# C-X-Lu/Replication-of-Minute-Frequency-Factor

Measured on AMD Instinct MI355X. Metric: factor stock-days/sec (whole node) + % of HBM roofline, 5000×240min×2500d, higher is better.
Workload: dtype f64

## Files before the change

### replication-of-minute-frequency-factor_amd/csrc/mff_group.h

```cpp
#pragma once
#include <hip/hip_runtime.h>
#include <stdint.h>

#include "mff_wave.h"

namespace mff {
namespace g16 {

__device__ __forceinline__ int gi() { return (int)(threadIdx.x & 15u); }
__device__ __forceinline__ int gbase() { return (int)(threadIdx.x & 48u); }

constexpr int QP_XOR1 = 0xB1;
constexpr int QP_XOR2 = 0x4E;
constexpr int ROW_SHR = 0x110;
constexpr int ROW_SHL = 0x100;
constexpr int ROW_MIRROR = 0x140;
constexpr int ROW_HALF_MIRROR = 0x141;
constexpr int K = 16;

template <int CTRL>
__device__ __forceinline__ int dpp_i(int x) {
  return __builtin_amdgcn_mov_dpp(x, CTRL, 0xF, 0xF, true);
}
template <int CTRL>
__device__ __forceinline__ uint32_t dpp_u(uint32_t x) { return (uint32_t)dpp_i<CTRL>((int)x); }
template <int CTRL>
__device__ __forceinline__ float dpp_f(float x) { return __int_as_float(dpp_i<CTRL>(__float_as_int(x))); }
template <int CTRL>
__device__ __forceinline__ double dpp_d(double x) {
  const uint64_t b = dbits(x);
  const uint32_t lo = (uint32_t)dpp_i<CTRL>((int)(uint32_t)b);
  const uint32_t hi = (uint32_t)dpp_i<CTRL>((int)(uint32_t)(b >> 32));
  return bitsd(((uint64_t)hi << 32) | lo);
}
template <int CTRL>
__device__ __forceinline__ uint64_t dpp_u64(uint64_t b) {
  const uint32_t lo = (uint32_t)dpp_i<CTRL>((int)(uint32_t)b);
  const uint32_t hi = (uint32_t)dpp_i<CTRL>((int)(uint32_t)(b >> 32));
  return ((uint64_t)hi << 32) | lo;
}

template <int CTRL>
__device__ __forceinline__ float dppT(float x) { return dpp_f<CTRL>(x); }
template <int CTRL>
__device__ __forceinline__ double dppT(double x) { return dpp_d<CTRL>(x); }
template <int CTRL>
__device__ __forceinline__ uint32_t dppT(uint32_t x) { return dpp_u<CTRL>(x); }

__device__ __forceinline__ double gsum(double x) {
  x += dpp_d<QP_XOR1>(x);
  x += dpp_d<QP_XOR2>(x);
  x += dpp_d<ROW_HALF_MIRROR>(x);
  x += dpp_d<ROW_MIRROR>(x);
  return x;
}
__device__ __forceinline__ double gprod(double x) {
  x *= dpp_d<QP_XOR1>(x);
  x *= dpp_d<QP_XOR2>(x);
  x *= dpp_d<ROW_HALF_MIRROR>(x);
  x *= dpp_d<ROW_MIRROR>(x);
  return x;
}
__device__ __forceinline__ int gsum_i(int x) {
  x += dpp_i<QP_XOR1>(x);
  x += dpp_i<QP_XOR2>(x);
  x += dpp_i<ROW_HALF_MIRROR>(x);
  x += dpp_i<ROW_MIRROR>(x);
  return x;
}
__device__ __forceinline__ uint32_t gsum_u(uint32_t x) { return (uint32_t)gsum_i((int)x); }
__device__ __forceinline__ int gmin_i(int x) {
  x = min(x, dpp_i<QP_XOR1>(x));
  x = min(x, dpp_i<QP_XOR2>(x));
  x = min(x, dpp_i<ROW_HALF_MIRROR>(x));
  x = min(x, dpp_i<ROW_MIRROR>(x));
  return x;
}
__device__ __forceinline__ int gmax_i(int x) {
  x = max(x, dpp_i<QP_XOR1>(x));
  x = max(x, dpp_i<QP_XOR2>(x));
  x = max(x, dpp_i<ROW_HALF_MIRROR>(x));
  x = max(x, dpp_i<ROW_MIRROR>(x));
  return x;
}
__device__ __forceinline__ bool gany(bool b) { return gmax_i(b ? 1 : 0) != 0; }

__device__ __forceinline__ double gscan_incl(double x) {
  x += dpp_d<ROW_SHR + 1>(x);
  x += dpp_d<ROW_SHR + 2>(x);
  x += dpp_d<ROW_SHR + 4>(x);
  x += dpp_d<ROW_SHR + 8>(x);
  return x;
}
__device__ __forceinline__ uint32_t gscan_incl_u(uint32_t x) {
  x += dpp_u<ROW_SHR + 1>(x);
  x += dpp_u<ROW_SHR + 2>(x);
  x += dpp_u<ROW_SHR + 4>(x);
  x += dpp_u<ROW_SHR + 8>(x);
  return x;
}
__device__ __forceinline__ double gscan_excl(double x) { return dpp_d<ROW_SHR + 1>(gscan_incl(x)); }
__device__ __forceinline__ uint32_t gscan_excl_u(uint32_t x) { return dpp_u<ROW_SHR + 1>(gscan_incl_u(x)); }

template <typename T>
__device__ __forceinline__ void carry_left(T v, bool h, T& cv, bool& ch) {
  uint32_t hh = h ? 1u : 0u;
#pragma unroll
  for (int step = 0; step < 4; ++step) {
    T ov;
    uint32_t oh;
    if (step == 0) { ov = dppT<ROW_SHR + 1>(v); oh = dpp_u<ROW_SHR + 1>(hh); }
    if (step == 1) { ov = dppT<ROW_SHR + 2>(v); oh = dpp_u<ROW_SHR + 2>(hh); }
    if (step == 2) { ov = dppT<ROW_SHR + 4>(v); oh = dpp_u<ROW_SHR + 4>(hh); }
    if (step == 3) { ov = dppT<ROW_SHR + 8>(v); oh = dpp_u<ROW_SHR + 8>(hh); }
    if (!hh && oh) { v = ov; hh = 1u; }
  }
  cv = dppT<ROW_SHR + 1>(v);
  ch = dpp_u<ROW_SHR + 1>(hh) != 0u;
}
template <typename T>
__device__ __forceinline__ void carry_right(T v, bool h, T& cv, bool& ch) {
  uint32_t hh = h ? 1u : 0u;
#pragma unroll
  for (int step = 0; step < 4; ++step) {
    T ov;
    uint32_t oh;
    if (step == 0) { ov = dppT<ROW_SHL + 1>(v); oh = dpp_u<ROW_SHL + 1>(hh); }
    if (step == 1) { ov = dppT<ROW_SHL + 2>(v); oh = dpp_u<ROW_SHL + 2>(hh); }
    if (step == 2) { ov = dppT<ROW_SHL + 4>(v); oh = dpp_u<ROW_SHL + 4>(hh); }
    if (step == 3) { ov = dppT<ROW_SHL + 8>(v); oh = dpp_u<ROW_SHL + 8>(hh); }
    if (!hh && oh) { v = ov; hh = 1u; }
  }
  cv = dppT<ROW_SHL + 1>(v);
  ch = dpp_u<ROW_SHL + 1>(hh) != 0u;
}

__device__ __forceinline__ int bpermi(int src_lane, int v) { return __builtin_amdgcn_ds_bpermute(src_lane << 2, v); }
__device__ __forceinline__ float bpermf(int src_lane, float v) { return __int_as_float(bpermi(src_lane, __float_as_int(v))); }
__device__ __forceinline__ uint32_t bpermu(int src_lane, uint32_t v) { return (uint32_t)bpermi(src_lane, (int)v); }
__device__ __forceinline__ double bpermd(int src_lane, double v) {
  const uint64_t b = dbits(v);
  const uint32_t lo = (uint32_t)bpermi(src_lane, (int)(uint32_t)b);
  const uint32_t hi = (uint32_t)bpermi(src_lane, (int)(uint32_t)(b >> 32));
  return bitsd(((uint64_t)hi << 32) | lo);
}

__device__ __forceinline__ uint32_t blend_u(bool c, uint32_t a, uint32_t b) {
  const uint32_t m = 0u - (uint32_t)c;
  return (a & m) | (b & ~m);
}
__device__ __forceinline__ uint32_t pick(const uint32_t (&x)[K], int k) {
  uint32_t t = x[0];
#pragma unroll
  for (int j = 1; j < K; ++j) t = blend_u(k == j, x[j], t);
  return t;
}
__device__ __forceinline__ float pick(const float (&x)[K], int k) {
  uint32_t t = __float_as_uint(x[0]);
#pragma unroll
  for (int j = 1; j < K; ++j) t = blend_u(k == j, __float_as_uint(x[j]), t);
  return __uint_as_float(t);
}
__device__ __forceinline__ uint64_t pick(const uint64_t (&x)[K], int k) {
  uint32_t lo = (uint32_t)x[0], hi = (uint32_t)(x[0] >> 32);
#pragma unroll
  for (int j = 1; j < K; ++j) {
    lo = blend_u(k == j, (uint32_t)x[j], lo);
    hi = blend_u(k == j, (uint32_t)(x[j] >> 32), hi);
  }
  return ((uint64_t)hi << 32) | lo;
}
__device__ __forceinline__ float gval(const float (&x)[K], int m) {
  return bpermf(gbase() + (m >> 4), pick(x, m & 15));
}
__device__ __forceinline__ uint32_t gvalu(const uint32_t (&x)[K], int m) {
  return bpermu(gbase() + (m >> 4), pick(x, m & 15));
}
template <int M>
__device__ __forceinline__ float gvalc(const float (&x)[K]) {
  return bpermf(gbase() + (M >> 4), x[M & 15]);
}
__device__ __forceinline__ bool gpres(uint32_t pb, int m) {
  return (bpermu(gbase() + (m >> 4), pb) >> (m & 15)) & 1u;
}

__device__ __forceinline__ uint32_t present_bits(uint32_t pb, int k) { return (uint32_t)((int32_t)(pb << (31 - k)) >> 31); }
__device__ __forceinline__ uint32_t absent_bits(uint32_t pb, int k) { return ~present_bits(pb, k); }

__device__ __forceinline__ uint32_t rmask(int lo, int hi) {
  const int b0 = 16 * gi();
  int a = lo - b0, b = hi - b0;
  if (a < 0) a = 0;
  if (b > 15) b = 15;
  if (b < a) return 0u;
  return ((0xFFFFu >> (15 - b)) >> a) << a;
}
__device__ __forceinline__ int gfirst(uint32_t m) {
  const int v = m ? 16 * gi() + (int)__builtin_ctz(m) : (1 << 20);
  const int r = gmin_i(v);
  return r == (1 << 20) ? -1 : r;
}
__device__ __forceinline__ int glast(uint32_t m) {
  return gmax_i(m ? 16 * gi() + 31 - (int)__builtin_clz(m) : -1);
}
__device__ __forceinline__ int gcount(uint32_t m) { return gsum_i(__builtin_popcount(m)); }
__device__ __forceinline__ uint32_t gmax_u(uint32_t x) {
  x = max(x, dpp_u<QP_XOR1>(x));
  x = max(x, dpp_u<QP_XOR2>(x));
  x = max(x, dpp_u<ROW_HALF_MIRROR>(x));
  x = max(x, dpp_u<ROW_MIRROR>(x));
  return x;
}
__device__ __forceinline__ uint32_t gmin_u(uint32_t x) {
  x = min(x, dpp_u<QP_XOR1>(x));
  x = min(x, dpp_u<QP_XOR2>(x));
  x = min(x, dpp_u<ROW_HALF_MIRROR>(x));
  x = min(x, dpp_u<ROW_MIRROR>(x));
  return x;
}

constexpr int QP_XOR3 = 0x1B;
constexpr int ROW_ROR8 = 0x128;

template <int CTRL>
__device__ __forceinline__ uint32_t dpp_full(uint32_t x) {
  return (uint32_t)__builtin_amdgcn_mov_dpp((int)x, CTRL, 0xF, 0xF, false);
}
__device__ __forceinline__ uint32_t swz_xor4(uint32_t x) {
  return (uint32_t)__builtin_amdgcn_ds_swizzle((int)x, 0x1F | (4 << 10));
}
template <int M>
__device__ __forceinline__ uint32_t gpartner(uint32_t x) {
  return (uint32_t)__builtin_amdgcn_ds_swizzle((int)x, 0x1F | (M << 10));
}
template <int M, int LB, bool FLIP>
__device__ __forceinline__ void gcross(uint32_t (&a)[K]) {
  const uint32_t bound = (gi() & LB) == 0 ? 0u : 0xFFFFFFFFu;
  uint32_t p[K];
#pragma unroll
  for (int k = 0; k < K; ++k) p[k] = gpartner<M>(a[FLIP ? K - 1 - k : k]);
#pragma unroll
  for (int k = 0; k < K; ++k) asm("v_med3_u32 %0, %1, %2, %3" : "=v"(a[k]) : "v"(a[k]), "v"(p[k]), "v"(bound));
}
template <int J, bool FLIP>
__device__ __forceinline__ void glocal(uint32_t (&a)[K]) {
#pragma unroll
  for (int k = 0; k < K; ++k) {
    const int o = FLIP ? (k ^ (2 * J - 1)) : (k ^ J);
    if (o > k) {
      const uint32_t x = a[k], y = a[o];
      a[k] = min(x, y);
      a[o] = max(x, y);
    }
  }
}
__device__ __forceinline__ void glocal_tail(uint32_t (&a)[K]) {
  glocal<8, false>(a);
  glocal<4, false>(a);
  glocal<2, false>(a);
  glocal<1, false>(a);
}
__device__ __forceinline__ void gsort16_lane(uint32_t (&a)[K]) {
  constexpr int8_t net[60][2] = {
      {0, 13}, {1, 12}, {2, 15}, {3, 14}, {4, 8}, {5, 6}, {7, 11}, {9, 10},
      {0, 5}, {1, 7}, {2, 9}, {3, 4}, {6, 13}, {8, 14}, {10, 15}, {11, 12},
      {0, 1}, {2, 3}, {4, 5}, {6, 8}, {7, 9}, {10, 11}, {12, 13}, {14, 15},
      {0, 2}, {1, 3}, {4, 10}, {5, 11}, {6, 7}, {8, 9}, {12, 14}, {13, 15},
      {1, 2}, {3, 12}, {4, 6}, {5, 7}, {8, 10}, {9, 11}, {13, 14},
      {1, 4}, {2, 6}, {5, 8}, {7, 10}, {9, 13}, {11, 14},
      {2, 4}, {3, 6}, {9, 12}, {11, 13},
// ... 22 lines not shown
```

### replication-of-minute-frequency-factor_amd/csrc/mff_stage1g.hip

```cpp
#include <stdlib.h>
#include <string.h>

#include <type_traits>

#include "../../include/mff.h"
#include "mff_group.h"
#include "mff_fmath.h"
#include "mff_stats.h"
#include "mff_internal.h"

namespace mff {

int launch_w64(const float* const fld[5], const uint32_t* valid, int S, int D, const int32_t* ids, int nf,
               double* val, uint8_t* state, double* pdfq, const int* list, const int* list_count,
               uint32_t fam_mask, int list_grid, hipStream_t st, uint32_t* lvl_count = nullptr,
               uint64_t* lvl_key = nullptr, uint8_t* lvl_w = nullptr);
int launch_serial(const float* const fld[5], const uint32_t* valid, int S, int D, const int8_t* row,
                  uint32_t fam, double* val, uint8_t* state, const uint32_t* ord_th, hipStream_t st);

constexpr int kGIter = 1;
constexpr int kGWaves = 5;
constexpr int kExactGrid = 1024;

namespace g16 {

constexpr int NB = 256;

struct GArgs {
  const float* fld[5];
  const uint32_t* mask;
  double* val;
  uint8_t* state;
  double* pdfq;
  uint32_t* lvl_count;
  uint64_t* lvl_key;
  uint8_t* lvl_w;
  int* fb_list;
  int* fb_count;
  uint32_t fam_exact;
  uint32_t* ord_th;
  int S, D;
  uint32_t fam;
  int8_t row[NF];
};

struct Res {
  double r[4];
  uint32_t st;
  __device__ __forceinline__ void put(int f, double x, uint32_t s) {
    if (gi() == (f & 15)) {
      const int q = f >> 4;
      r[q] = x;
      st = (st & ~(0xFFu << (8 * q))) | (s << (8 * q));
    }
  }
  __device__ __forceinline__ void val(int f, double x) { put(f, x, MFF_STATE_VALUE); }
  __device__ __forceinline__ void null(int f) { put(f, 0.0, MFF_STATE_NULL); }
};

__device__ __forceinline__ double gmin_d(double x) {
  x = fmin(x, dpp_d<QP_XOR1>(x));
  x = fmin(x, dpp_d<QP_XOR2>(x));
  x = fmin(x, dpp_d<ROW_HALF_MIRROR>(x));
  x = fmin(x, dpp_d<ROW_MIRROR>(x));
  return x;
}
__device__ __forceinline__ double gmax_d(double x) {
  x = fmax(x, dpp_d<QP_XOR1>(x));
  x = fmax(x, dpp_d<QP_XOR2>(x));
  x = fmax(x, dpp_d<ROW_HALF_MIRROR>(x));
  x = fmax(x, dpp_d<ROW_MIRROR>(x));
  return x;
}

__device__ __forceinline__ void opaque(float& x) { asm("" : "+v"(x)); }
__device__ __forceinline__ void opaque(double& x) { asm("" : "+v"(x)); }
__device__ __forceinline__ void opaque(uint32_t& x) { asm("" : "+v"(x)); }
template <typename T>
__device__ __forceinline__ void fresh(T (&x)[K]) {
#pragma unroll
  for (int k = 0; k < K; ++k) opaque(x[k]);
}

__device__ __forceinline__ void lds_fence() {
  __builtin_amdgcn_fence(__ATOMIC_RELEASE, "wavefront");
  __builtin_amdgcn_wave_barrier();
  __builtin_amdgcn_fence(__ATOMIC_ACQUIRE, "wavefront");
}

__device__ __forceinline__ uint32_t xor_lane(uint32_t x, int lj) { return (uint32_t)__shfl_xor((int)x, lj, 16); }
__device__ __forceinline__ uint64_t xor_lane(uint64_t x, int lj) {
  const uint32_t lo = xor_lane((uint32_t)x, lj), hi = xor_lane((uint32_t)(x >> 32), lj);
  return ((uint64_t)hi << 32) | lo;
}

template <typename T>
__device__ __forceinline__ void gsort256(T (&a)[K]) {
  const int g = gi();
#pragma unroll
  for (int size = 2; size <= 256; size <<= 1) {
#pragma unroll
    for (int j = size >> 1; j > 0; j >>= 1) {
      if (j >= 16) {
        const int lj = j >> 4;
        const bool lower = (g & lj) == 0;
        const bool up = ((16 * g) & size) == 0;
#pragma unroll
        for (int k = 0; k < K; ++k) {
          const T p = xor_lane(a[k], lj);
          const T mn = a[k] < p ? a[k] : p, mx = a[k] < p ? p : a[k];
          a[k] = (lower == up) ? mn : mx;
        }
      } else {
#pragma unroll
        for (int k = 0; k < K; ++k) {
          if ((k & j) == 0) {
            const bool up = ((16 * g + k) & size) == 0;
            const T x = a[k], y = a[k | j];
            const T mn = x < y ? x : y, mx = x < y ? y : x;
            a[k] = up ? mn : mx;
            a[k | j] = up ? mx : mn;
          }
        }
      }
    }
  }
}

[[maybe_unused]] constexpr uint32_t G_HL = F_OLS | F_MOMH;
constexpr uint32_t G_ORD = F_ORD | F_ORDV;
constexpr uint32_t G_LVL = F_LVL | F_PDF;
constexpr uint32_t kGroups[2] = {G_ORD, G_LVL};
constexpr uint32_t G_OL = G_ORD | G_LVL;

template <uint32_t SET>
__global__ __launch_bounds__(256, kGWaves) void k_stage1g(GArgs a) {
  constexpr int SW = (SET & F_OLS) ? 2 * NB : 2 * NBAR;
  __shared__ __attribute__((aligned(16))) uint64_t scratch[16][SW / 2 + 8];
  const int lane = lane_id();
  const int wave = threadIdx.x >> 6;
  const int grp = lane >> 4;
  const int g = gi();
  const int gb = gbase();
  uint64_t* scr = scratch[wave * 4 + grp];
  double* scr_d = reinterpret_cast<double*>(scr);
  const uint32_t fam = a.fam & SET;
  const int ntile = (a.S + 16 * kGIter - 1) / (16 * kGIter);
  const int d = blockIdx.x / ntile;
  const int s0 = (blockIdx.x % ntile) * (16 * kGIter);
  const size_t plane = (size_t)a.D * a.S;

  for (int it = 0; it < kGIter; ++it) {
    const int s = s0 + it * 16 + wave * 4 + grp;
    const bool act = s < a.S;
    const size_t sd = (size_t)d * a.S + (act ? s : 0);
    const bool ln = act && g < 15;

    uint32_t pb = 0;
    if (ln) {
      const uint32_t w = a.mask[sd * 8 + (g >> 1)];
      pb = (w >> (16 * (g & 1))) & 0xFFFFu;
    }
    const int n = gcount(pb);
    Res R;
    R.r[0] = R.r[1] = R.r[2] = R.r[3] = 0.0;
    R.st = 0u;
    double qv = qnan();
    uint32_t emitL = 0u, emitB = 0u;
    float emitC = 1.0f;

    if (n > 0) {
      float o[K], h[K], lo[K], c[K];
      uint32_t v[K];
      auto load = [&](int f, float (&x)[K], float dflt) {
        if (ln) {
          const float4* p4 = reinterpret_cast<const float4*>(a.fld[f] + sd * NBAR + 16 * g);
#pragma unroll
          for (int q = 0; q < 4; ++q) {
            const float4 t = p4[q];
            x[4 * q + 0] = t.x; x[4 * q + 1] = t.y; x[4 * q + 2] = t.z; x[4 * q + 3] = t.w;
          }
        } else {
#pragma unroll
          for (int k = 0; k < K; ++k) x[k] = dflt;
        }
      };
      constexpr uint32_t needO = F_SEG | F_MOMR | F_TRD;
      constexpr uint32_t needHL = F_OLS | F_MOMH;
      constexpr uint32_t needC = F_SEG | F_MOMR | F_SUMC | F_CORR | F_LVL | F_PDF | F_TRD;
      constexpr uint32_t needV = F_ORD | F_MOMV | F_SUMC | F_SUMV | F_CORR | F_LVL | F_PDF | F_ORDV | F_TRD;
      static_assert(!(needO & ~kFieldFams[0]) && !(needHL & ~(kFieldFams[1] & kFieldFams[2])) &&
                        !(needC & ~kFieldFams[3]) && !(needV & ~kFieldFams[4]),
                    "k_stage1g loads a field for a family kFieldFams does not list");
      auto loadv = [&](uint32_t (&x)[K]) {
        if (ln) {
          const uint4* p4 = reinterpret_cast<const uint4*>(a.fld[4] + sd * NBAR + 16 * g);
#pragma unroll
          for (int q = 0; q < 4; ++q) {
            const uint4 t = p4[q];
            x[4 * q + 0] = t.x; x[4 * q + 1] = t.y; x[4 * q + 2] = t.z; x[4 * q + 3] = t.w;
          }
#pragma unroll
          for (int k = 0; k < K; ++k) x[k] &= present_bits(pb, k);
        } else {
#pragma unroll
          for (int k = 0; k < K; ++k) x[k] = 0u;
        }
      };
      auto sanitize = [&](float (&x)[K], float dflt) {
#pragma unroll
        for (int k = 0; k < K; ++k) {
          if (dflt == 0.0f)
            x[k] = bitsf(fbits(x[k] + 0.0f) & present_bits(pb, k));
          else
            x[k] = ((pb >> k) & 1u) ? x[k] + 0.0f : dflt;
        }
      };
      if (fam & needHL) {
        load(1, h, 1.0f);
        load(2, lo, 1.0f);
        sanitize(h, 1.0f);
        sanitize(lo, 1.0f);
      }
      const int fb = gfirst(pb), lb = glast(pb);

      if (fam & F_OLS) {
        const double x0a = (double)gval(lo, fb), y0a = (double)gval(h, fb);
        const float ln0 = dpp_f<ROW_SHL + 1>(lo[0]), hn0 = dpp_f<ROW_SHL + 1>(h[0]);
        const uint32_t pn0 = dpp_u<ROW_SHL + 1>(pb) & 1u;
        double tx = 0, ty = 0, txx = 0, tyy = 0, txy = 0, q15x = 0, q15y = 0, q15xx = 0, q15yy = 0, q15xy = 0;
        uint32_t tpk = 0, q15pk = 0;
#pragma unroll
        for (int k = 0; k < K; ++k) {
          const bool pk = (pb >> k) & 1u;
          const bool pnx = (k < 15) ? ((pb >> (k + 1)) & 1u) : (pn0 != 0u);
          const float lnx = (k < 15) ? lo[k + 1] : ln0, hnx = (k < 15) ? h[k + 1] : hn0;
          const double dx = pk ? (double)lo[k] - x0a : 0.0, dy = pk ? (double)h[k] - y0a : 0.0;
          const uint32_t pkv = (pk ? 1u : 0u) | ((pk && pnx && lo[k] != lnx) ? 0x100u : 0u) |
                               ((pk && pnx && h[k] != hnx) ? 0x10000u : 0u);
          tx += dx; ty += dy; txx += dx * dx; tyy += dy * dy; txy += dx * dy; tpk += pkv;
          if (k == 15) { q15x = dx; q15y = dy; q15xx = dx * dx; q15yy = dy * dy; q15xy = dx * dy; q15pk = pkv; }
        }
        double Rx = gscan_excl(tx), Ry = gscan_excl(ty), Rxx = gscan_excl(txx), Ryy = gscan_excl(tyy),
               Rxy = gscan_excl(txy);
        uint32_t Rpk = gscan_excl_u(tpk);
        const double E15x = Rx + tx, E15y = Ry + ty, E15xx = Rxx + txx, E15yy = Ryy + tyy, E15xy = Rxy + txy;
        const uint32_t E15pk = Rpk + tpk;
        double x0 = x0a, y0 = y0a;
        opaque(x0);
        opaque(y0);
#pragma unroll
        for (int k = 0; k < K; ++k) { opaque(lo[k]); opaque(h[k]); }
        double H1x = 0, H1y = 0, H1xx = 0, H1yy = 0, H1xy = 0, H2x = 0, H2y = 0, H2xx = 0, H2yy = 0, H2xy = 0;
        uint32_t H1pk = 0, H2pk = 0;
        double sq = 0, scs = 0, scr = 0, bsum = 0, blast = 0;
        int lastT = -1, wq = 0;
        uint32_t wmask = 0;
#pragma unroll
        for (int k = 0; k < K; ++k) {
          const bool pk = (pb >> k) & 1u;
          const bool pnx = (k < 15) ? ((pb >> (k + 1)) & 1u) : (pn0 != 0u);
          const float lnx = (k < 15) ? lo[k + 1] : ln0, hnx = (k < 15) ? h[k + 1] : hn0;
          const double dx = pk ? (double)lo[k] - x0 : 0.0, dy = pk ? (double)h[k] - y0 : 0.0;
          const uint32_t chx = (pk && pnx && lo[k] != lnx) ? 1u : 0u;
          const uint32_t chy = (pk && pnx && h[k] != hnx) ? 1u : 0u;
          Rx += dx; Ry += dy; Rxx += dx * dx; Ryy += dy * dy; Rxy += dx * dy;
          Rpk += (pk ? 1u : 0u) | (chx << 8) | (chy << 16);
          double bx, by, bxx, byy, bxy;
          uint32_t bpk;
          if (k >= 2) {
            const int src = gb + (g >= 3 ? g - 3 : 0);
            bx = bpermd(src, H2x); by = bpermd(src, H2y); bxx = bpermd(src, H2xx);
            byy = bpermd(src, H2yy); bxy = bpermd(src, H2xy); bpk = bpermu(src, H2pk);
            if (g < 3) { bx = by = bxx = byy = bxy = 0.0; bpk = 0u; }
          } else {
            const int src = gb + (g >= 4 ? g - 4 : 0);
            const double ex = (k == 0) ? E15x - q15x : E15x, ey = (k == 0) ? E15y - q15y : E15y;
            const double exx = (k == 0) ? E15xx - q15xx : E15xx, eyy = (k == 0) ? E15yy - q15yy : E15yy;
            const double exy = (k == 0) ? E15xy - q15xy : E15xy;
            const uint32_t epk = (k == 0) ? E15pk - q15pk : E15pk;
            bx = bpermd(src, ex); by = bpermd(src, ey); bxx = bpermd(src, exx);
            byy = bpermd(src, eyy); bxy = bpermd(src, exy); bpk = bpermu(src, epk);
            if (g < 4) { bx = by = bxx = byy = bxy = 0.0; bpk = 0u; }
          }
          H2x = H1x; H2y = H1y; H2xx = H1xx; H2yy = H1yy; H2xy = H1xy; H2pk = H1pk;
          H1x = Rx; H1y = Ry; H1xx = Rxx; H1yy = Ryy; H1xy = Rxy; H1pk = Rpk;
          const int t = 16 * g + k;
          const uint32_t cnt = (Rpk & 0xffu) - (bpk & 0xffu);
          const uint32_t cxw = ((Rpk >> 8) & 0xffu) - ((bpk >> 8) & 0xffu) - chx;
          const uint32_t cyw = ((Rpk >> 16) & 0xffu) - ((bpk >> 16) & 0xffu) - chy;
          const bool okw = ln && t >= 49 && cnt == 50u;
          if (okw) {
            const double Sx = Rx - bx, Sy = Ry - by, Sxx = Rxx - bxx, Syy = Ryy - byy, Sxy = Rxy - bxy;
            const bool cx = cxw == 0u, cy = cyw == 0u;
            const double vx = cx ? 0.0 : (Sxx - Sx * Sx * 0.02) * 0.02;
            const double vy = cy ? 0.0 : (Syy - Sy * Sy * 0.02) * 0.02;
            const double cv = (cx || cy) ? 0.0 : (Sxy - Sx * Sy * 0.02) * 0.02;
            double beta;
            if (vx != 0.0) beta = cv / vx;
            else beta = (y0 + Sy * 0.02) / (x0 + Sx * 0.02);
            const double prod = vx * vy;
            if (prod != 0.0) {
              const double ip = 1.0 / prod;
              sq += sqrt(cv) * ip;
              scs += cv * cv * ip;
              scr += cv * sqrt(prod) * ip;
              ++wq;
            }
            scr_d[t] = beta;
            bsum += beta;
            blast = beta;
            lastT = t;
            wmask |= 1u << k;
          }
          __builtin_amdgcn_sched_barrier(0);
        }
        const int W = gcount(wmask);
        if (W > 0) {
          lds_fence();
          const int fT = gfirst(wmask), lT = gmax_i(lastT);
          const double b0 = scr_d[fT];
          const double bl = bpermd(gb + (lT >> 4), blast);
          double d1 = 0.0, d2 = 0.0;
#pragma unroll
          for (int k = 0; k < K; ++k)
            if ((wmask >> k) & 1u) {
              const double dd = scr_d[16 * g + k] - b0;
              d1 += dd;
              d2 += dd * dd;
            }
          d1 = gsum(d1);
          d2 = gsum(d2);
          const int Wq = gsum_i(wq);
          const double Sq = gsum(sq), Scs = gsum(scs), Scr = gsum(scr);
          const double bmean = b0 + d1 / (double)W;
          double bstd = 0.0;
          const bool has_std = W >= 2;
          if (has_std) bstd = sqrt((d2 - d1 * d1 / (double)W) / (double)(W - 1));
          (void)bsum;
          if (has_std && tot_ne(bstd, 0.0) && Wq > 0)
            R.val(5, (Sq / (double)Wq) * (bl - bmean) / bstd);
          else
            R.val(5, 0.0);
          R.val(6, Wq > 0 ? Scs / (double)Wq : 0.0);
          R.val(7, Wq > 0 ? Scr / (double)Wq : 0.0);
          R.val(8, bmean);
          R.val(9, (has_std && tot_gt(bstd, 0.0)) ? (bl - bmean) / bstd : bmean);
          lds_fence();
        }
      }

      __builtin_amdgcn_sched_barrier(0);
      if (fam & F_MOMH) {
        fresh(h);
        fresh(lo);

        const double x0 = (double)gval(h, fb) / (double)gval(lo, fb);
        double s1 = 0, s2 = 0;
#pragma unroll
        for (int k = 0; k < K; ++k)
          if ((pb >> k) & 1u) {
            const double dd = (double)h[k] / (double)lo[k] - x0;
            s1 += dd;
            s2 += dd * dd;
          }
        RawMom m{gsum(s1), gsum(s2), 0, 0, n};
        double sdv;
        if (std1_raw(m, m.s1 == 0.0 && m.s2 == 0.0, sdv)) R.val(15, sdv); else R.null(15);
      }

      __builtin_amdgcn_sched_barrier(0);
      double sumv = 0.0;
      if (fam & needV) {
        loadv(v);
        double t = 0.0;
#pragma unroll
        for (int k = 0; k < K; ++k) t += (double)v[k];
        sumv = gsum(t);
      }
      if (fam & needC) {
        load(3, c, 1.0f);
        if (fam & needC & ~(F_LVL | F_PDF)) sanitize(c, 1.0f);
      }
      if (fam & needO) {
        load(0, o, 1.0f);
        sanitize(o, 1.0f);
      }

      if (fam & (F_ORD | F_ORDV)) {
        fresh(v);

        uint32_t key[K];
#pragma unroll
        for (int k = 0; k < K; ++k) key[k] = v[k] | absent_bits(pb, k);
        gsort256u(key);
        uint32_t* so = reinterpret_cast<uint32_t*>(scr);
#pragma unroll
        for (int k = 0; k < K; ++k) so[16 * k + g] = key[k];
        lds_fence();
        const int e = g < 10 ? n - 1 - g
                    : g == 10 ? (n >= 50 ? n - 50 : 0)
                    : g == 11 ? (n >= 20 ? n - 20 : 0)
                    : (n >= 50 ? 49 : n - 1);
        const uint32_t xe = (e >= 0 && g < 13) ? so[((e & 15) << 4) | (e >> 4)] : 0u;
        lds_fence();
        if ((fam & F_ORD) && a.ord_th && g >= 10 && g < 13 && act) {
          const size_t pl = (size_t)a.D * a.S;
          a.ord_th[(size_t)(g - 10) * pl + sd] = xe;
        }
        if (fam & F_ORDV) {
          const double t10 = gsum(g < 10 ? (double)xe : 0.0);
          const double t5 = gsum(g < 5 ? (double)xe : 0.0);
          R.val(47, t10 / sumv);
          R.val(48, t5 / sumv);
          R.val(49, t5 / sumv);
        }
      }

      if (fam & (F_MOMR | F_TRD)) {
        fresh(c);
        fresh(o);
        fresh(v);

        const double x0 = (double)gval(c, fb) / (double)gval(o, fb) - 1.0;
        double s1 = 0, s2 = 0, s3 = 0, s4 = 0;
        double u1 = 0, u2 = 0, umn = __builtin_inf(), umx = -__builtin_inf();
        double w1 = 0, w2 = 0, wmn = __builtin_inf(), wmx = -__builtin_inf();
        uint32_t upm = 0, dnm = 0;
        double vT20 = 0, vT50 = 0, rT20 = 0, rT50 = 0, vH20 = 0, vH50 = 0, a20 = 0, n20 = 0, q20 = 0, a50 = 0;
#pragma unroll
        for (int k = 0; k < K; ++k) {
          const bool pk = (pb >> k) & 1u;
          const int m = 16 * g + k;
          const double q = (double)c[k] / (double)o[k];
          const double r = q - 1.0;
          if (pk) {
            const double dd = r - x0, d2 = dd * dd;
            s1 += dd; s2 += d2; s3 += d2 * dd; s4 += d2 * d2;
            if (tot_gt(r, 0.0)) { upm |= 1u << k; u1 += dd; u2 += d2; umn = fmin(umn, r); umx = fmax(umx, r); }
            if (tot_lt(r, 0.0)) { dnm |= 1u << k; w1 += dd; w2 += d2; wmn = fmin(wmn, r); wmx = fmax(wmx, r); }
            const double vk = (double)v[k];
            if (m >= 220) { vT20 += vk; rT20 += vk * r; }
            if (m >= 190) { vT50 += vk; rT50 += vk * r; }
            if (m <= 50) {
              const double iw = 1.0 / vk;
              const double ta = r * iw;
              vH50 += vk; a50 += ta;
              if (m <= 20) {
                vH20 += vk; a20 += ta;
                n20 += (r < 0.0 ? -r : 0.0) * iw;
                q20 += (r > 0.0 ? r : 0.0) * iw;
              }
            }
          }
        }
        if (fam & F_MOMR) {
          RawMom m{gsum(s1), gsum(s2), gsum(s3), gsum(s4), n};
          double sdr;
          const bool has_sdr = std1_raw(m, m.s1 == 0.0 && m.s2 == 0.0, sdr);
          if (has_sdr) R.val(16, sdr); else R.null(16);
          const int nu = gcount(upm), nd = gcount(dnm);
          const double U1 = gsum(u1), U2 = gsum(u2), Umn = gmin_d(umn), Umx = gmax_d(umx);
          const double D1 = gsum(w1), D2 = gsum(w2), Dmn = gmin_d(wmn), Dmx = gmax_d(wmx);
          double sup = 0.0, sdn = 0.0;
          std1_raw(RawMom{U1, U2, 0, 0, nu}, Umn == Umx, sup);
          std1_raw(RawMom{D1, D2, 0, 0, nd}, Dmn == Dmx, sdn);
          R.val(17, sup);
          R.val(19, sdn);
          if (has_sdr) { R.val(18, sup / sdr); R.val(20, sdn / sdr); }
          else { R.null(18); R.null(20); }
          double sk, ku;
          skew_kurt(m, sk, ku);
          R.val(21, sk);
          R.val(22, ku);
          R.val(23, sk / ku);
        }
        if (fam & F_TRD) {
// ... 145 lines not shown
            for (int i = 0; i < 3; ++i)
#pragma unroll
              for (int j = 0; j < 5; ++j) P[i][j] = 0.0;
            float cp = cpv;
            uint32_t vp = vpv;
            bool h_ = hp;
#pragma unroll
            for (int k = 0; k < K; ++k) {
              if ((pb >> k) & 1u) {
                const double ck = (double)c[k], vk = (double)v[k];
                double dx = ck - x2, dy = vk - y2;
                P[0][0] += dx; P[0][1] += dy; P[0][2] += dx * dx; P[0][3] += dy * dy; P[0][4] += dx * dy;
                if (h_) {
                  const double pc = (ck - (double)cp) / (double)cp;
                  dx = pc - x1; dy = vk - y1;
                  P[1][0] += dx; P[1][1] += dy; P[1][2] += dx * dx; P[1][3] += dy * dy; P[1][4] += dx * dy;
                  dx = ck - x3; dy = (double)vp - y3;
                  P[2][0] += dx; P[2][1] += dy; P[2][2] += dx * dx; P[2][3] += dy * dy; P[2][4] += dx * dy;
                }
                cp = c[k]; vp = v[k]; h_ = true;
              }
            }
            fin(35, n, P[0][0], P[0][1], P[0][2], P[0][3], P[0][4]);
            fin(33, n - 1, P[1][0], P[1][1], P[1][2], P[1][3], P[1][4]);
            fin(36, n - 1, P[2][0], P[2][1], P[2][2], P[2][3], P[2][4]);
          }
          if (nzc > 0) {
            double P[2][5];
#pragma unroll
            for (int i = 0; i < 2; ++i)
#pragma unroll
              for (int j = 0; j < 5; ++j) P[i][j] = 0.0;
            float czp = cpz;
            uint32_t vzp = vpz;
            bool hz_ = hz;
#pragma unroll
            for (int k = 0; k < K; ++k) {
              if (((nzm >> k) & 1u)) {
                const double ck = (double)c[k], vk = (double)v[k];
                if (hz_) {
                  const double pcz = (ck - (double)czp) / (double)czp;
                  const double pvz = (vk - (double)vzp) / (double)vzp;
                  double dx = pcz - x5, dy = pvz - y5;
                  P[0][0] += dx; P[0][1] += dy; P[0][2] += dx * dx; P[0][3] += dy * dy; P[0][4] += dx * dy;
                  dx = ck - x6;
                  P[1][0] += dx; P[1][1] += dy; P[1][2] += dx * dx; P[1][3] += dy * dy; P[1][4] += dx * dy;
                }
                czp = c[k]; vzp = v[k]; hz_ = true;
              }
            }
            fin(34, nzc - 1, P[0][0], P[0][1], P[0][2], P[0][3], P[0][4]);
            fin(38, nzc - 1, P[1][0], P[1][1], P[1][2], P[1][3], P[1][4]);
          }
          {
            double a0 = 0, a1 = 0, a2 = 0, a3 = 0, a4 = 0;
            uint32_t fvv = 0u;
#pragma unroll
            for (int k = K - 1; k >= 0; --k)
              if ((pb >> k) & 1u) fvv = v[k];
            uint32_t vn;
            bool hn;
            carry_right(fvv, pb != 0u, vn, hn);
#pragma unroll
            for (int k = K - 1; k >= 0; --k)
              if ((pb >> k) & 1u) {
                if (hn) {
                  const double dx = (double)c[k] - x4, dy = (double)vn - y4;
                  a0 += dx; a1 += dy; a2 += dx * dx; a3 += dy * dy; a4 += dx * dy;
                }
                vn = v[k];
                hn = true;
              }
            fin(37, n - 1, a0, a1, a2, a3, a4);
          }
        }
      }

      if (fam & (F_LVL | F_PDF)) {
        fresh(c);
        fresh(v);
        uint32_t cmx = 0u, cmn = 0xffffffffu;
#pragma unroll
        for (int k = 0; k < K; ++k) {
          cmx = max(cmx, fbits(c[k]) & present_bits(pb, k));
          cmn = min(cmn, fbits(c[k]) | absent_bits(pb, k));
        }
        const bool ok = sumv < 4294967296.0;
        cmx = gmax_u(cmx);
        cmn = gmin_u(cmn);
        const float clastf = gval(c, lb);
        bool fast = !gany(!ok);
        const int e0 = 16 * g;
        uint32_t cw[K], vv[K], cbase = cmx;
        const bool wide = cmx - cmn >= (1u << 24);
        if (wide) {
          if (g == 0 && !(grid_skip(a.mask[sd * 8 + 7]) & (F_LVL | F_PDF))) {
            const int idx = atomicAdd(a.fb_count, 1);
            a.fb_list[idx] = (int)((uint32_t)sd | 0x80000000u);
          }
#pragma unroll
          for (int k = 0; k < K; ++k) { cw[k] = 0u; vv[k] = 0u; }
        } else {
          uint32_t* sv = reinterpret_cast<uint32_t*>(scr);
          uint32_t key[K];
#pragma unroll
          for (int k = 0; k < K; ++k) {
            const uint32_t slot = (uint32_t)(16 * k + g);
            sv[slot] = v[k];
            key[k] = ((cmx - fbits(c[k])) << 8) | slot | absent_bits(pb, k);
          }
          gsort256u(key);
          lds_fence();
#pragma unroll
          for (int k = 0; k < K; ++k) {
            cw[k] = key[k] >> 8;
            vv[k] = sv[key[k] & 0xffu];
          }
          lds_fence();
        }
        const int nin = min(max(n - e0, 0), K);
        const uint32_t validm = (uint32_t)((1u << nin) - 1u);
        const uint32_t nextw = dpp_u<ROW_SHL + 1>(cw[0]);
        uint32_t diffm = 0u, tv = 0u;
#pragma unroll
        for (int k = 0; k < K; ++k) {
          const uint32_t wn = k < K - 1 ? cw[k + 1] : nextw;
          diffm |= (cw[k] != wn ? 1u : 0u) << k;
          tv += vv[k];
        }
        const uint32_t lastm = (n - 1 >= e0 && n - 1 < e0 + K) ? 1u << (n - 1 - e0) : 0u;
        const uint32_t endm = (diffm | lastm) & validm;
        const int L = gcount(endm);
        if (!wide && a.lvl_key) {
          emitL = (uint32_t)L;
          emitC = clastf;
          emitB = cbase;
        }
        if (!wide) {
          uint32_t* lv = reinterpret_cast<uint32_t*>(scr);
          uint32_t* lc = lv + NBAR;
          uint32_t cum = gscan_excl_u(tv);
          int li = (int)gscan_excl_u((uint32_t)__builtin_popcount(endm));
#pragma unroll
          for (int k = 0; k < K; ++k) {
            cum += vv[k];
            if ((endm >> k) & 1u) {
              lv[li] = cum;
              lc[li] = (cw[k] << 8) | (uint32_t)(e0 + k);
              ++li;
            }
          }
          lds_fence();
          const uint32_t Sv = (uint32_t)sumv;
          const double inv = 1.0 / sumv;
          const double x0 = (double)lv[0] * inv;
          double s1 = 0, s2 = 0, s3 = 0, s4 = 0;
          if (fam & F_LVL) {
            for (int l = g; l < L; l += 16) {
              const uint32_t V = lv[l] - (l > 0 ? lv[l - 1] : 0u);
              const double dd = (double)V * inv - x0, d2 = dd * dd;
              s1 += dd; s2 += d2; s3 += d2 * dd; s4 += d2 * d2;
            }
          }
          if (fast && (fam & F_LVL)) {
            RawMom m{gsum(s1), gsum(s2), gsum(s3), gsum(s4), L};
            double sk, ku;
            skew_kurt(m, sk, ku);
            if (!(sumv > 0.0)) sk = ku = qnan();
            R.val(39, ku);
            R.val(40, sk);
            R.val(41, sk);
          }
          if (fast && (fam & F_PDF)) {
            const uint32_t kt = g == 0 ? 12u : g == 1 ? 14u : g == 2 ? 16u : g == 3 ? 18u : 19u;
            const uint32_t sq20 = Sv / 20u, sr20 = Sv - 20u * sq20;
            const uint32_t b = kt * sr20;
            const uint32_t bq = b / 20u;
            const uint32_t T = kt * sq20 + bq;
            int e = 0;
#pragma unroll
            for (int st = 128; st >= 1; st >>= 1)
              if (e + st <= L && lv[e + st - 1] <= T) e += st;
            const bool tie = g < 5 && b == 20u * bq && e > 0 && lv[e - 1] == T;
            if (gany(tie) && Sv != 0u) fast = false;
            if (Sv == 0u) e = 0;
            if (g < 5 && e < L) qv = fdiv_f32in(clastf, bitsf(cbase - (lc[e] >> 8)));
          }
          lds_fence();
        }
        if (!fast && !wide && (fam & (a.fam_exact))) {
          if (g == 0 && !(grid_skip(a.mask[sd * 8 + 7]) & (F_LVL | F_PDF))) {
            const int idx = atomicAdd(a.fb_count, 1);
            a.fb_list[idx] = (int)sd;
          }
        }
        if (fam & F_PDF) {
          if (!fast) qv = qnan();
#pragma unroll
          for (int t = 0; t < 5; ++t) R.null(PDF0 + t);
        }
      }
    }

    const uint32_t skip = act ? grid_skip(a.mask[sd * 8 + 7]) : 0u;
    if (skip & F_PDF) emitL = 0u;
    const bool emit = a.lvl_key != nullptr;
    uint32_t lpreA = 0u, lpreB = 0u, gA = 0u;
    uint64_t lwb = 0ull;
    if (emit) {
      const uint32_t* lc = reinterpret_cast<const uint32_t*>(scr) + NBAR;
      const uint64_t ksplit = pdf_split_key(a.lvl_count, a.D);
      auto key_at = [&](int l) {
        return dbits(fdiv_f32in(emitC, bitsf(emitB - (lc[l] >> 8)))) | 0x8000000000000000ull;
      };
      const int pb = 16 * g + 15;
      const bool lb1 = pb < (int)emitL && key_at(pb) < ksplit;
      const uint32_t c1 = (uint32_t)__popc((uint32_t)(__ballot(lb1) >> gbase()) & 0xFFFFu);
      const int pw = 16 * (int)c1 + g;
      const bool lb2 = pw < (int)emitL && key_at(pw) < ksplit;
      gA = 16u * c1 + (uint32_t)__popc((uint32_t)(__ballot(lb2) >> gbase()) & 0xFFFFu);
      const uint32_t nB = emitL - gA;
      const uint32_t a0 = (uint32_t)__builtin_amdgcn_readlane((int)gA, 0);
      const uint32_t a1 = (uint32_t)__builtin_amdgcn_readlane((int)gA, 16);
      const uint32_t a2 = (uint32_t)__builtin_amdgcn_readlane((int)gA, 32);
      const uint32_t a3 = (uint32_t)__builtin_amdgcn_readlane((int)gA, 48);
      const uint32_t b0 = (uint32_t)__builtin_amdgcn_readlane((int)nB, 0);
      const uint32_t b1 = (uint32_t)__builtin_amdgcn_readlane((int)nB, 16);
      const uint32_t b2 = (uint32_t)__builtin_amdgcn_readlane((int)nB, 32);
      const uint32_t b3 = (uint32_t)__builtin_amdgcn_readlane((int)nB, 48);
      lpreA = grp == 0 ? 0u : grp == 1 ? a0 : grp == 2 ? a0 + a1 : a0 + a1 + a2;
      lpreB = grp == 0 ? 0u : grp == 1 ? b0 : grp == 2 ? b0 + b1 : b0 + b1 + b2;
      const uint64_t tot = (uint64_t)(a0 + a1 + a2 + a3) | ((uint64_t)(b0 + b1 + b2 + b3) << 32);
      if (lane == 0 && tot != 0ull)
        lwb = atomicAdd(reinterpret_cast<unsigned long long*>(a.lvl_count) + d, (unsigned long long)tot);
    }

    if (act && skip != ~0u) {
      auto store = [&](auto kept) {
#pragma unroll
        for (int q = 0; q < 4; ++q) {
          const int f = 16 * q + g;
          if (f < NF) {
            const int row = a.row[f];
            if (row >= 0 && (!decltype(kept)::value || !(kFamOf(f) & skip))) {
              a.val[(size_t)row * plane + sd] = R.r[q];
              a.state[(size_t)row * plane + sd] = (uint8_t)((R.st >> (8 * q)) & 0xFFu);
            }
          }
        }
      };
      if (__builtin_amdgcn_ballot_w64(skip != 0u) == 0ull) store(std::false_type());
      else store(std::true_type());
      if (a.pdfq && g < 5 && !(skip & F_PDF)) {
        a.pdfq[(size_t)g * plane + sd] = qv;
      }
    }
    if (emit) {
      const uint64_t wb = ((uint64_t)__builtin_amdgcn_readfirstlane((int)(uint32_t)(lwb >> 32)) << 32) |
                          (uint32_t)__builtin_amdgcn_readfirstlane((int)(uint32_t)lwb);
      const uint32_t baseA = (uint32_t)wb + lpreA, baseB = (uint32_t)(wb >> 32) + lpreB;
      const uint32_t* lc = reinterpret_cast<const uint32_t*>(scr) + NBAR;
      const size_t capd = pdf_day_cap(a.S);
      uint64_t* kd = a.lvl_key + (size_t)d * capd;
      uint8_t* wd = a.lvl_w + (size_t)d * capd;
      for (int l = g; l < (int)emitL; l += 16) {
        const uint32_t cwb = lc[l];
        const uint32_t ee = cwb & 0xFFu;
        const uint32_t ep = l > 0 ? (lc[l - 1] & 0xFFu) : 0xFFFFFFFFu;
        const size_t at = (uint32_t)l < gA ? (size_t)(baseA + (uint32_t)l)
                                          : capd - 1 - (size_t)(baseB + (uint32_t)l - gA);
        kd[at] = dbits(fdiv_f32in(emitC, bitsf(emitB - (cwb >> 8)))) | 0x8000000000000000ull;
        wd[at] = (uint8_t)(ee - ep);
      }
      lds_fence();
    }
  }
}

}
}

using namespace mff;

extern "C" size_t mff_stage1_workspace_bytes(int S, int D) {
  return 256 + (size_t)S * (size_t)D * (sizeof(int) + 3 * sizeof(uint32_t));
}

namespace mff {
size_t pdf_levels_split(int S, int D, size_t* off_key, size_t* off_w) {
  const size_t cap = pdf_day_cap(S) * (size_t)D;
  *off_key = (pdf_koff(D) + 8 + 255) & ~(size_t)255;
  *off_w = *off_key + cap * 8;
  return *off_w + cap;
}
}

extern "C" size_t mff_pdf_levels_bytes(int S, int D) {
  size_t a, b;
  return pdf_levels_split(S, D, &a, &b);
}

static int stage1_parts(const float* open, const float* high, const float* low, const float* close,
                        const uint32_t* volume, const uint32_t* valid, int S, int D, const int32_t* factor_ids,
                        int nf, double* val, uint8_t* state, double* pdf_query, void* pdf_levels,
                        void* workspace, void* stream, int part) {
  clear_error();
  MFF_REQUIRE(part == 1 || part == 2 || part == 3 || part == 4 || part == 10 || part == 11 || part == 17 ||
                  part == 32 || part == 64 || part == 129 || part == 145,
              "mff_stage1_part: part=%d must be 1, 2, 3, 4, 10, 11, 17, 32, 64, 129 or 145", part);
  MFF_REQUIRE(S > 0 && D > 0, "mff_stage1: S=%d D=%d must be positive", S, D);
  MFF_REQUIRE((long long)S * D < (1ll << 31), "mff_stage1: S*D must be < 2^31");
  MFF_REQUIRE(nf > 0 && nf <= NF, "mff_stage1: nf=%d out of range", nf);
  MFF_REQUIRE(factor_ids != nullptr, "mff_stage1: factor_ids is NULL");
  MFF_REQUIRE(valid && val && state, "mff_stage1: NULL device buffer");
  MFF_REQUIRE(workspace != nullptr, "mff_stage1: workspace is NULL (mff_stage1_workspace_bytes)");
  const float* fld[5] = {open, high, low, close, reinterpret_cast<const float*>(volume)};
  g16::GArgs a;
  memset(&a, 0, sizeof(a));
  for (int f = 0; f < 5; ++f) a.fld[f] = fld[f];
  a.mask = valid; a.val = val; a.state = state; a.pdfq = pdf_query;
  a.S = S; a.D = D;
  a.fam_exact = ~0u;
  for (int i = 0; i < NF; ++i) a.row[i] = -1;
  for (int r = 0; r < nf; ++r) {
    const int id = factor_ids[r];
    MFF_REQUIRE(id >= 0 && id < NF, "mff_stage1: factor id %d out of range", id);
    MFF_REQUIRE(a.row[id] < 0, "mff_stage1: factor id %d requested twice", id);
    a.row[id] = (int8_t)r;
    a.fam |= kFactorFamily[id];
  }
  static_assert(rows_fams(MFF_ROWS_KEEP | (1u << MFF_ROWS_NULL_SHIFT)) == kFieldFams[0], "open");
  static_assert(rows_fams(MFF_ROWS_KEEP | (16u << MFF_ROWS_NULL_SHIFT)) == kFieldFams[4], "volume");
  static_assert(rows_fams(MFF_ROWS_LISTED) == ~0u && grid_skip(0u) == 0u, "listed whole / not listed");
  for (int f = 0; f < 5; ++f)
    MFF_REQUIRE(!(a.fam & kFieldFams[f]) || fld[f] != nullptr, "mff_stage1: field plane %d required", f);
  MFF_REQUIRE(!(a.fam & F_PDF) || (pdf_query != nullptr && pdf_levels != nullptr),
              "mff_stage1: doc_pdf requested but pdf_query / pdf_levels is NULL");
  hipStream_t st = as_stream(stream);
  int* cnt = reinterpret_cast<int*>(workspace);
  a.fb_count = cnt;
  a.fb_list = reinterpret_cast<int*>(reinterpret_cast<char*>(workspace) + 256);
  a.ord_th = reinterpret_cast<uint32_t*>(reinterpret_cast<char*>(workspace) + 256 + (size_t)S * D * sizeof(int));
  const char* impl = getenv("MFF_STAGE1_IMPL");
  const bool w64 = impl && strcmp(impl, "w64") == 0;
  const long long nblk = (long long)((S + 16 * kGIter - 1) / (16 * kGIter)) * D;
  auto group_launch = [&](int gi) -> int {
    const uint32_t set = gi < 2 ? g16::kGroups[gi] : g16::G_OL;
    if (!(a.fam & set)) return 0;
    g16::GArgs b = a;
    for (int i = 0; i < NF; ++i)
      if (!(kFactorFamily[i] & set)) b.row[i] = -1;
    if (!(set & F_PDF)) b.pdfq = nullptr;
    if (gi == 0) hipLaunchKernelGGL(g16::k_stage1g<g16::G_ORD>, dim3((unsigned)nblk), dim3(256), 0, st, b);
    else if (gi == 1) hipLaunchKernelGGL(g16::k_stage1g<g16::G_LVL>, dim3((unsigned)nblk), dim3(256), 0, st, b);
    else hipLaunchKernelGGL(g16::k_stage1g<g16::G_OL>, dim3((unsigned)nblk), dim3(256), 0, st, b);
    MFF_LAUNCH_CHECK();
    return 0;
  };
  if (a.fam & F_PDF) {
    size_t ok, ow;
    pdf_levels_split(S, D, &ok, &ow);
    char* base = reinterpret_cast<char*>(pdf_levels);
    a.lvl_count = reinterpret_cast<uint32_t*>(base);
    a.lvl_key = reinterpret_cast<uint64_t*>(base + ok);
    a.lvl_w = reinterpret_cast<uint8_t*>(base + ow);
  }
  if (part == 32) {
    if (w64 || !(a.fam & (F_LVL | F_PDF))) return 0;
    return launch_w64(fld, valid, S, D, factor_ids, nf, val, state, pdf_query, a.fb_list, cnt, F_LVL | F_PDF, kExactGrid,
                      st, a.lvl_count, a.lvl_key, a.lvl_w);
  }
  if (part & 65) {
    if (!(part & 128)) {
      if (a.fam & F_PDF) {
        MFF_HIP(hipMemsetAsync(a.lvl_count, 0, (size_t)D * 8, st));
        if (pdf_split_init(a.lvl_count, D, st) != 0) return -2;
      }
      MFF_HIP(hipMemsetAsync(cnt, 0, sizeof(int), st));
    }
    if (part == 64) return 0;
  }
  if (part & 1) {
    if (w64) {
      const int rc = launch_w64(fld, valid, S, D, factor_ids, nf, val, state, pdf_query, nullptr, nullptr, ~0u, 0, st);
      if (rc != 0 || !(a.fam & F_PDF)) return rc;
      g16::GArgs b = a;
      for (int i = 0; i < NF; ++i) b.row[i] = -1;
      b.pdfq = nullptr;
      b.fam = F_PDF;
      b.fam_exact = 0u;
      hipLaunchKernelGGL(g16::k_stage1g<g16::G_LVL>, dim3((unsigned)nblk), dim3(256), 0, st, b);
      MFF_LAUNCH_CHECK();
      return launch_w64(fld, valid, S, D, factor_ids, nf, val, state, pdf_query, a.fb_list, cnt, F_PDF, kExactGrid, st,
                        a.lvl_count, a.lvl_key, a.lvl_w);
    }
    int rc = group_launch((a.fam & g16::G_ORD) && (a.fam & (F_LVL | F_PDF)) ? 2 : 1);
    if (rc != 0) return rc;
    if ((a.fam & (F_LVL | F_PDF)) && !(part & 16)) {
      rc = launch_w64(fld, valid, S, D, factor_ids, nf, val, state, pdf_query, a.fb_list, cnt,
                      F_LVL | F_PDF, kExactGrid, st, a.lvl_count, a.lvl_key, a.lvl_w);
      if (rc != 0) return rc;
    }
  }
  constexpr uint32_t kHL = F_OLS | F_MOMH;
  if (part & 4) {
    if (w64) return 0;
    return launch_serial(fld, valid, S, D, a.row, a.fam & kHL, val, state, a.ord_th, st);
  }
  if ((part & 2) && !w64) {
    if (!((a.fam & g16::G_ORD) && (a.fam & (F_LVL | F_PDF)))) {
      const int rc = group_launch(0);
      if (rc != 0) return rc;
    }
    return launch_serial(fld, valid, S, D, a.row, (part & 8) ? a.fam & ~kHL : a.fam, val, state, a.ord_th, st);
  }
  return 0;
}

extern "C" int mff_stage1(const float* open, const float* high, const float* low, const float* close,
                          const uint32_t* volume, const uint32_t* valid, int S, int D, const int32_t* factor_ids,
                          int nf, double* val, uint8_t* state, double* pdf_query, void* pdf_levels,
                          void* workspace, void* stream) {
  return stage1_parts(open, high, low, close, volume, valid, S, D, factor_ids, nf, val, state, pdf_query,
                      pdf_levels, workspace, stream, 3);
}

extern "C" int mff_stage1_part(const float* open, const float* high, const float* low, const float* close,
                               const uint32_t* volume, const uint32_t* valid, int S, int D,
                               const int32_t* factor_ids, int nf, double* val, uint8_t* state,
                               double* pdf_query, void* pdf_levels, void* workspace, void* stream, int part) {
  return stage1_parts(open, high, low, close, volume, valid, S, D, factor_ids, nf, val, state, pdf_query,
                      pdf_levels, workspace, stream, part);
}
```

Baseline: 308.3 million.

## Micro-optimize stage1g group kernel: swizzle sums, unconditional loads, precomputed row offsets

Replaces the DPP-based 16-lane double sum with ds_swizzle butterflies. Removes the per-lane branch around field loads by clamping the load address, then masking absent bars with select-based predicates. It also precomputes 64-bit row offsets on the host so stores skip a multiply, prunes store lanes at compile time per family set, and uses inline asm to build the bit mask in the level detection. Several of these are independent micro-tweaks. They trade DPP for LDS-path swizzles and add kernel argument size.

```diff
diff --git a/replication-of-minute-frequency-factor_amd/csrc/mff_group.h b/replication-of-minute-frequency-factor_amd/csrc/mff_group.h
--- a/replication-of-minute-frequency-factor_amd/csrc/mff_group.h
+++ b/replication-of-minute-frequency-factor_amd/csrc/mff_group.h
@@ -47,11 +47,19 @@
 template <int CTRL>
 __device__ __forceinline__ uint32_t dppT(uint32_t x) { return dpp_u<CTRL>(x); }
 
+template <int M>
+__device__ __forceinline__ double swz_d(double x) {
+  const uint64_t b = dbits(x);
+  const uint32_t lo = (uint32_t)__builtin_amdgcn_ds_swizzle((int)(uint32_t)b, 0x1F | (M << 10));
+  const uint32_t hi = (uint32_t)__builtin_amdgcn_ds_swizzle((int)(uint32_t)(b >> 32), 0x1F | (M << 10));
+  return bitsd(((uint64_t)hi << 32) | lo);
+}
+
 __device__ __forceinline__ double gsum(double x) {
-  x += dpp_d<QP_XOR1>(x);
-  x += dpp_d<QP_XOR2>(x);
-  x += dpp_d<ROW_HALF_MIRROR>(x);
-  x += dpp_d<ROW_MIRROR>(x);
+  x += swz_d<1>(x);
+  x += swz_d<2>(x);
+  x += swz_d<7>(x);
+  x += swz_d<15>(x);
   return x;
 }
 __device__ __forceinline__ double gprod(double x) {
@@ -186,6 +194,7 @@
 
 __device__ __forceinline__ uint32_t present_bits(uint32_t pb, int k) { return (uint32_t)((int32_t)(pb << (31 - k)) >> 31); }
 __device__ __forceinline__ uint32_t absent_bits(uint32_t pb, int k) { return ~present_bits(pb, k); }
+__device__ __forceinline__ bool has(uint32_t pb, int k) { return ((pb >> k) & 1u) != 0u; }
 
 __device__ __forceinline__ uint32_t rmask(int lo, int hi) {
   const int b0 = 16 * gi();
diff --git a/replication-of-minute-frequency-factor_amd/csrc/mff_stage1g.hip b/replication-of-minute-frequency-factor_amd/csrc/mff_stage1g.hip
--- a/replication-of-minute-frequency-factor_amd/csrc/mff_stage1g.hip
+++ b/replication-of-minute-frequency-factor_amd/csrc/mff_stage1g.hip
@@ -42,7 +42,15 @@
   int S, D;
   uint32_t fam;
   int8_t row[NF];
+  int64_t rowoff[NF];
 };
+
+__host__ __device__ constexpr uint32_t res_lanes(uint32_t held, int q) {
+  uint32_t m = 0u;
+  for (int l = 0; l < 16; ++l)
+    if (16 * q + l < NF && (kFamOf(16 * q + l) & held)) m |= 1u << l;
+  return m;
+}
 
 struct Res {
   double r[4];
@@ -172,17 +180,13 @@
     if (n > 0) {
       float o[K], h[K], lo[K], c[K];
       uint32_t v[K];
-      auto load = [&](int f, float (&x)[K], float dflt) {
-        if (ln) {
-          const float4* p4 = reinterpret_cast<const float4*>(a.fld[f] + sd * NBAR + 16 * g);
-#pragma unroll
-          for (int q = 0; q < 4; ++q) {
-            const float4 t = p4[q];
-            x[4 * q + 0] = t.x; x[4 * q + 1] = t.y; x[4 * q + 2] = t.z; x[4 * q + 3] = t.w;
-          }
-        } else {
-#pragma unroll
-          for (int k = 0; k < K; ++k) x[k] = dflt;
+      const size_t ldoff = sd * NBAR + 16 * min(g, 14);
+      auto load = [&](int f, float (&x)[K]) {
+        const float4* p4 = reinterpret_cast<const float4*>(a.fld[f] + ldoff);
+#pragma unroll
+        for (int q = 0; q < 4; ++q) {
+          const float4 t = p4[q];
+          x[4 * q + 0] = t.x; x[4 * q + 1] = t.y; x[4 * q + 2] = t.z; x[4 * q + 3] = t.w;
         }
       };
       constexpr uint32_t needO = F_SEG | F_MOMR | F_TRD;
@@ -193,19 +197,15 @@
                         !(needC & ~kFieldFams[3]) && !(needV & ~kFieldFams[4]),
                     "k_stage1g loads a field for a family kFieldFams does not list");
       auto loadv = [&](uint32_t (&x)[K]) {
-        if (ln) {
-          const uint4* p4 = reinterpret_cast<const uint4*>(a.fld[4] + sd * NBAR + 16 * g);
-#pragma unroll
-          for (int q = 0; q < 4; ++q) {
-            const uint4 t = p4[q];
-            x[4 * q + 0] = t.x; x[4 * q + 1] = t.y; x[4 * q + 2] = t.z; x[4 * q + 3] = t.w;
-          }
-#pragma unroll
-          for (int k = 0; k < K; ++k) x[k] &= present_bits(pb, k);
-        } else {
-#pragma unroll
-          for (int k = 0; k < K; ++k) x[k] = 0u;
-        }
+        const uint4* p4 = reinterpret_cast<const uint4*>(a.fld[4] + ldoff);
+#pragma unroll
+        for (int q = 0; q < 4; ++q) {
+          const uint4 t = p4[q];
+          x[4 * q + 0] = t.x; x[4 * q + 1] = t.y; x[4 * q + 2] = t.z; x[4 * q + 3] = t.w;
+        }
+        __builtin_amdgcn_sched_barrier(0);
+#pragma unroll
+        for (int k = 0; k < K; ++k) x[k] = has(pb, k) ? x[k] : 0u;
       };
       auto sanitize = [&](float (&x)[K], float dflt) {
 #pragma unroll
@@ -217,8 +217,8 @@
         }
       };
       if (fam & needHL) {
-        load(1, h, 1.0f);
-        load(2, lo, 1.0f);
+        load(1, h);
+        load(2, lo);
         sanitize(h, 1.0f);
         sanitize(lo, 1.0f);
       }
@@ -371,7 +371,7 @@
 
       __builtin_amdgcn_sched_barrier(0);
       double sumv = 0.0;
-      if (fam & needV) {
+      if (!(SET & ~needV) || (fam & needV)) {
         loadv(v);
         double t = 0.0;
 #pragma unroll
@@ -379,11 +379,11 @@
         sumv = gsum(t);
       }
       if (fam & needC) {
-        load(3, c, 1.0f);
+        load(3, c);
         if (fam & needC & ~(F_LVL | F_PDF)) sanitize(c, 1.0f);
       }
       if (fam & needO) {
-        load(0, o, 1.0f);
+        load(0, o);
         sanitize(o, 1.0f);
       }
 
@@ -392,7 +392,7 @@
 
         uint32_t key[K];
 #pragma unroll
-        for (int k = 0; k < K; ++k) key[k] = v[k] | absent_bits(pb, k);
+        for (int k = 0; k < K; ++k) key[k] = has(pb, k) ? v[k] : 0xffffffffu;
         gsort256u(key);
         uint32_t* so = reinterpret_cast<uint32_t*>(scr);
 #pragma unroll
@@ -704,8 +704,8 @@
         uint32_t cmx = 0u, cmn = 0xffffffffu;
 #pragma unroll
         for (int k = 0; k < K; ++k) {
-          cmx = max(cmx, fbits(c[k]) & present_bits(pb, k));
-          cmn = min(cmn, fbits(c[k]) | absent_bits(pb, k));
+          cmx = max(cmx, has(pb, k) ? fbits(c[k]) : 0u);
+          cmn = min(cmn, has(pb, k) ? fbits(c[k]) : 0xffffffffu);
         }
         const bool ok = sumv < 4294967296.0;
         cmx = gmax_u(cmx);
@@ -729,7 +729,7 @@
           for (int k = 0; k < K; ++k) {
             const uint32_t slot = (uint32_t)(16 * k + g);
             sv[slot] = v[k];
-            key[k] = ((cmx - fbits(c[k])) << 8) | slot | absent_bits(pb, k);
+            key[k] = has(pb, k) ? ((cmx - fbits(c[k])) << 8) | slot : 0xffffffffu;
           }
           gsort256u(key);
           lds_fence();
@@ -745,9 +745,12 @@
         const uint32_t nextw = dpp_u<ROW_SHL + 1>(cw[0]);
         uint32_t diffm = 0u, tv = 0u;
 #pragma unroll
-        for (int k = 0; k < K; ++k) {
+        for (int k = K - 1; k >= 0; --k) {
           const uint32_t wn = k < K - 1 ? cw[k + 1] : nextw;
-          diffm |= (cw[k] != wn ? 1u : 0u) << k;
+          asm("v_cmp_ne_u32_e32 vcc, %1, %2\n\tv_addc_co_u32_e32 %0, vcc, %0, %0, vcc"
+              : "+v"(diffm)
+              : "v"(cw[k]), "v"(wn)
+              : "vcc");
           tv += vv[k];
         }
         const uint32_t lastm = (n - 1 >= e0 && n - 1 < e0 + K) ? 1u << (n - 1 - e0) : 0u;
@@ -762,14 +765,14 @@
           uint32_t* lv = reinterpret_cast<uint32_t*>(scr);
           uint32_t* lc = lv + NBAR;
           uint32_t cum = gscan_excl_u(tv);
-          int li = (int)gscan_excl_u((uint32_t)__builtin_popcount(endm));
+          uint32_t* pl = lv + (int)gscan_excl_u((uint32_t)__builtin_popcount(endm));
 #pragma unroll
           for (int k = 0; k < K; ++k) {
             cum += vv[k];
             if ((endm >> k) & 1u) {
-              lv[li] = cum;
-              lc[li] = (cw[k] << 8) | (uint32_t)(e0 + k);
-              ++li;
+              pl[0] = cum;
+              pl[NBAR] = (cw[k] << 8) | (uint32_t)(e0 + k);
+              ++pl;
             }
           }
           lds_fence();
@@ -858,15 +861,18 @@
     }
 
     if (act && skip != ~0u) {
+      constexpr uint32_t held = SET & ~F_ORD;
       auto store = [&](auto kept) {
 #pragma unroll
         for (int q = 0; q < 4; ++q) {
-          const int f = 16 * q + g;
-          if (f < NF) {
-            const int row = a.row[f];
-            if (row >= 0 && (!decltype(kept)::value || !(kFamOf(f) & skip))) {
-              a.val[(size_t)row * plane + sd] = R.r[q];
-              a.state[(size_t)row * plane + sd] = (uint8_t)((R.st >> (8 * q)) & 0xFFu);
+          const uint32_t lanes = res_lanes(held, q);
+          if (lanes != 0u && ((lanes >> g) & 1u)) {
+            const int f = 16 * q + g;
+            const int64_t off = a.rowoff[f];
+            if (off >= 0 && (!decltype(kept)::value || !(kFamOf(f) & skip))) {
+              const size_t at = (size_t)off + sd;
+              a.val[at] = R.r[q];
+              a.state[at] = (uint8_t)((R.st >> (8 * q)) & 0xFFu);
             }
           }
         }
@@ -943,12 +949,13 @@
   a.mask = valid; a.val = val; a.state = state; a.pdfq = pdf_query;
   a.S = S; a.D = D;
   a.fam_exact = ~0u;
-  for (int i = 0; i < NF; ++i) a.row[i] = -1;
+  for (int i = 0; i < NF; ++i) { a.row[i] = -1; a.rowoff[i] = -1; }
   for (int r = 0; r < nf; ++r) {
     const int id = factor_ids[r];
     MFF_REQUIRE(id >= 0 && id < NF, "mff_stage1: factor id %d out of range", id);
     MFF_REQUIRE(a.row[id] < 0, "mff_stage1: factor id %d requested twice", id);
     a.row[id] = (int8_t)r;
+    a.rowoff[id] = (int64_t)r * S * D;
     a.fam |= kFactorFamily[id];
   }
   static_assert(rows_fams(MFF_ROWS_KEEP | (1u << MFF_ROWS_NULL_SHIFT)) == kFieldFams[0], "open");
@@ -971,7 +978,7 @@
     if (!(a.fam & set)) return 0;
     g16::GArgs b = a;
     for (int i = 0; i < NF; ++i)
-      if (!(kFactorFamily[i] & set)) b.row[i] = -1;
+      if (!(kFactorFamily[i] & set)) { b.row[i] = -1; b.rowoff[i] = -1; }
     if (!(set & F_PDF)) b.pdfq = nullptr;
     if (gi == 0) hipLaunchKernelGGL(g16::k_stage1g<g16::G_ORD>, dim3((unsigned)nblk), dim3(256), 0, st, b);
     else if (gi == 1) hipLaunchKernelGGL(g16::k_stage1g<g16::G_LVL>, dim3((unsigned)nblk), dim3(256), 0, st, b);
@@ -1007,7 +1014,7 @@
       const int rc = launch_w64(fld, valid, S, D, factor_ids, nf, val, state, pdf_query, nullptr, nullptr, ~0u, 0, st);
       if (rc != 0 || !(a.fam & F_PDF)) return rc;
       g16::GArgs b = a;
-      for (int i = 0; i < NF; ++i) b.row[i] = -1;
+      for (int i = 0; i < NF; ++i) { b.row[i] = -1; b.rowoff[i] = -1; }
       b.pdfq = nullptr;
       b.fam = F_PDF;
       b.fam_exact = 0u;
```

Result: no change. 311.3 million (median of 6 runs) (+1.0%).
